# sangaprabhav/HypTokenizer

Hardware: AMD Instinct MI355X
Metric: merge_steps_per_sec (higher is better)
Workload: dtype bf16 prefilter + f32 canonical

## Files before the change

### hyptokenizer_amd/csrc/hm_engine.hip

```cpp
#include "hm_common.h"

static thread_local std::string g_last_error;

int hm_fail(hm_engine* e, int code, const std::string& msg)
{
    g_last_error = msg;
    if (e) e->err = msg;
    return code;
}

#define HM_WIDTH(v) v,
static const int kSupportedNG[] = {HM_SCAN_NG_LIST(HM_WIDTH, HM_SCAN_WIDTHS_ALL)};
static const int kSupportedKC[] = {HM_SCAN_KC_LIST(HM_WIDTH, HM_SCAN_WIDTHS_ALL)};
#undef HM_WIDTH

static int hm_pick_kc(int d)
{
    const int need = (d + 4 + 7) / 8;
    for (int v : kSupportedKC)
        if (v >= need) return v;
    return -1;
}

static int hm_pick_ng(int d)
{
    const int need = (d + 3) / 4;
    for (int v : kSupportedNG)
        if (v >= need) return v;
    return -1;
}

extern "C" int hm_abi_version(void) { return HM_ABI_VERSION; }

#if defined(HM_TUNING)
static const char* const kKnobNames[] = {"chunk", "tail", "tail_div", "big_rows", "shape", "incr_topk", "kc_even", "phases", "ph_share0", "ph_share1", "ph_share2", "ph_share3", "ph_share4",
                                        "ph_div1", "ph_div2", "ph_div3", "ph_div4", "ph_div5", "pipeline", "pipe_fault_at", "pipeline_pairs", "dyn", "dyn_slots", "head", "head_force", "head_ring", "head_span", "argmin_col_begin"};
#endif
static std::map<std::string, double> g_default_knobs;

static int hm_apply_knob(hm_engine* e, const char* name, double v)
{
    const std::string k = name ? name : "";
    if (k == "chunk") { if (!(v >= 4 && v <= 4096)) return HM_E_ARG; e->plan.chunk_f32 = e->plan.chunk_bf16 = (int)v; }
    else if (k == "tail") { if (!(v >= 0.0 && v <= 0.9)) return HM_E_ARG; e->plan.tail_fraction = v; }
    else if (k == "tail_div") { if (!(v >= 1 && v <= 16)) return HM_E_ARG; e->plan.tail_div = (int)v; }
    else if (k == "big_rows") { if (!(v >= 0)) return HM_E_ARG; e->plan.big_min_rows = (int64_t)v; }
    else if (k == "shape") { if (!(v >= -1 && v <= 4)) return HM_E_ARG; e->plan.force_shape = (int)v; }
    else if (k == "incr_topk") e->incremental_topk = v != 0.0;
    else if (k == "phases") { if (!(v >= 1 && v <= HM_SCAN_PHASES)) return HM_E_ARG; e->plan.phases = (int)v; }
    else if (k.size() == 9 && k.compare(0, 8, "ph_share") == 0 && k[8] >= '0' && k[8] < '0' + HM_SCAN_PHASES - 1) { if (!(v >= 0.0 && v <= 1.0)) return HM_E_ARG; e->plan.ph_share[k[8] - '0'] = v; }
    else if (k.size() == 7 && k.compare(0, 6, "ph_div") == 0 && k[6] >= '1' && k[6] < '0' + HM_SCAN_PHASES) { if (!(v >= 1 && v <= 64)) return HM_E_ARG; e->plan.ph_div[k[6] - '0'] = (int)v; }
    else if (k == "dyn_slots") { if (!(v >= 0 && v <= 65536)) return HM_E_ARG; e->dyn_slots = (int)v; }
    else if (k == "head") { if (!(v == 0.0 || v == (double)HM_SCAN_HEAD)) return HM_E_ARG; e->head = (int)v; }
    else if (k == "head_force") e->head_force = v != 0.0;
    else if (k == "head_ring") { if (!(v >= 0 && v < HM_SCAN_RINGS && v == (double)(int)v)) return HM_E_ARG; e->head_ring = (int)v; }
    else if (k == "head_span") { if (!(v == 1.0 || v == 2.0)) return HM_E_ARG; e->head_span = (int)v; }
    else if (k == "argmin_col_begin") { if (!(v >= 0)) return HM_E_ARG; e->argmin_col_begin = (int64_t)v; }
    else if (k == "expect_head_bad") { if (e->h == nullptr || (e->h->head_bad != 0u) != (v != 0.0)) return HM_E_STATE; return HM_OK; }
    else if (k == "dyn") e->dyn_queue = v != 0.0;
    else if (k == "pipeline") e->pipeline = v != 0.0;
    else if (k == "pipe_fault_at") e->pipe_fault_at = (int)v;
    else if (k == "exact_search") e->force_exact = v != 0.0;
    else if (k == "pipeline_pairs") { if (!(v >= 0)) return HM_E_ARG; e->pipeline_min_pairs = (int64_t)v; }
    else if (k == "kc_even") {
        if (e->img16 != nullptr) return HM_E_STATE;
        if (v != 0.0 && (e->KC & 1)) { e->KC += 1; e->RB16 = 16 * hm_row16_chunks(e->KC); }
    }
    else return HM_E_ARG;
    e->st.disarm();
    return HM_OK;
}

extern "C" int hm_debug_set_knob(hm_engine* e, const char* name, double value)
{
    if (!e) return hm_fail(nullptr, HM_E_ARG, "hm_debug_set_knob: engine is NULL");
    const int rc = hm_apply_knob(e, name, value);
    return rc ? hm_fail(e, rc, "hm_debug_set_knob: unknown knob or value out of range") : HM_OK;
}

extern "C" int hm_debug_set_default_knob(const char* name, double value, int clear)
{
    const std::string k = name ? name : "";
    if (clear) {
        if (k.empty()) { g_default_knobs.clear(); return hm_graph_default_knob(nullptr, 0.0, 1); }
        if (hm_graph_owns_knob(name)) return hm_graph_default_knob(name, 0.0, 1);
        g_default_knobs.erase(k);
        return HM_OK;
    }
    if (const int gk = hm_graph_default_knob(name, value, 0); gk <= 0)
        return gk ? hm_fail(nullptr, gk, "hm_debug_set_default_knob: unknown knob or value out of range") : HM_OK;
    hm_engine probe;
    const int rc = hm_apply_knob(&probe, name, value);
    if (rc) return hm_fail(nullptr, rc, "hm_debug_set_default_knob: unknown knob or value out of range");
    g_default_knobs[k] = value;
    return HM_OK;
}

extern "C" const char* hm_last_error(const hm_engine* e)
{
    if (e && !e->err.empty()) return e->err.c_str();
    return g_last_error.c_str();
}

static int hm_engine_alloc(hm_engine* e)
{
    const int device = e->device;
    HM_HIP(hipSetDevice(device));
    {
        int cus = 0;
        if (hipDeviceGetAttribute(&cus, hipDeviceAttributeMultiprocessorCount, device) == hipSuccess && cus > 0) e->n_cu = cus;
    }
    HM_HIP(hipMalloc(&e->img, sizeof(float) * (size_t)e->rows_alloc * e->RS));
    HM_HIP(hipMemset(e->img, 0, sizeof(float) * (size_t)e->rows_alloc * e->RS));
    HM_HIP(hipMalloc(&e->img16, (size_t)e->rows_alloc * e->RB16));
    HM_HIP(hipMemset(e->img16, 0, (size_t)e->rows_alloc * e->RB16));
    HM_HIP(hipMalloc(&e->ent, sizeof(uint4) * (size_t)e->ent_cap));
    HM_HIP(hipMalloc(&e->ent2, sizeof(uint4) * (size_t)e->ent_cap));
    HM_HIP(hipMalloc(&e->sorted, sizeof(uint4) * (size_t)e->sorted_cap));
    HM_HIP(hipMalloc(&e->d_prev, sizeof(uint4) * (size_t)e->sorted_cap));
    HM_HIP(hipMalloc(&e->d_batch, sizeof(int32_t) * 3 * HM_BATCH_MAX));
    HM_HIP(hipHostMalloc(&e->h_batch, sizeof(int32_t) * 3 * HM_BATCH_MAX, hipHostMallocDefault));
    HM_HIP(hipEventCreateWithFlags(&e->ev_batch, hipEventDisableTiming));
    HM_HIP(hipMalloc(&e->d_ctr, sizeof(uint32_t) * 8));
    HM_HIP(hipMemset(e->d_ctr, 0, sizeof(uint32_t) * 8));
    HM_HIP(hipMalloc(&e->d_rmax2_mem, sizeof(uint32_t) * 4));
    HM_HIP(hipMemset(e->d_rmax2_mem, 0, sizeof(uint32_t) * 4));
    e->d_rmax2 = e->d_rmax2_mem;
    HM_HIP(hipMalloc(&e->d_ctr64, sizeof(unsigned long long) * 8));
    HM_HIP(hipMemset(e->d_ctr64, 0, sizeof(unsigned long long) * 8));
    HM_HIP(hipMalloc(&e->d_queue, 256));
    HM_HIP(hipMemset(e->d_queue, 0, 256));
    HM_HIP(hipMalloc(&e->d_rowkey, sizeof(unsigned long long) * 3));
    HM_HIP(hipMemset(e->d_rowkey, 0xff, sizeof(unsigned long long) * 3));
    HM_HIP(hipMalloc(&e->d_seed, sizeof(ArgminSeed)));
    HM_HIP(hipMemset(e->d_seed, 0, sizeof(ArgminSeed)));
    HM_HIP(hipMalloc(&e->d_rec, 2 * sizeof(ArgminRec)));
    HM_HIP(hipMalloc(&e->d_loop_recs, HM_LOOP_MAX_STEPS * sizeof(ArgminRec)));
    HM_HIP(hipMalloc(&e->d_loop, sizeof(LoopState)));
// ... 222 lines not shown
```

### hyptokenizer_amd/csrc/hm_scan.hip

```cpp
#include <type_traits>

#include "hm_common.h"

#pragma clang fp contract(off)


template <int CNT>
__device__ __forceinline__ void hm_dma_group(const char* src, uint32_t dst)
{
    uint32_t keep;
    if constexpr (CNT == 4)
        asm volatile("s_mov_b32 %0, m0\n\ts_mov_b32 m0, %2\n\ts_nop 0\n\tglobal_load_lds_dwordx4 %1, off\n\t"
                     "global_load_lds_dwordx4 %1, off offset:1024\n\tglobal_load_lds_dwordx4 %1, off offset:2048\n\t"
                     "global_load_lds_dwordx4 %1, off offset:3072\n\ts_mov_b32 m0, %0"
                     : "=&s"(keep) : "v"(src), "s"(dst) : "memory");
    else if constexpr (CNT == 3)
        asm volatile("s_mov_b32 %0, m0\n\ts_mov_b32 m0, %2\n\ts_nop 0\n\tglobal_load_lds_dwordx4 %1, off\n\t"
                     "global_load_lds_dwordx4 %1, off offset:1024\n\tglobal_load_lds_dwordx4 %1, off offset:2048\n\t"
                     "s_mov_b32 m0, %0"
                     : "=&s"(keep) : "v"(src), "s"(dst) : "memory");
    else if constexpr (CNT == 2)
        asm volatile("s_mov_b32 %0, m0\n\ts_mov_b32 m0, %2\n\ts_nop 0\n\tglobal_load_lds_dwordx4 %1, off\n\t"
                     "global_load_lds_dwordx4 %1, off offset:1024\n\ts_mov_b32 m0, %0"
                     : "=&s"(keep) : "v"(src), "s"(dst) : "memory");
    else
        asm volatile("s_mov_b32 %0, m0\n\ts_mov_b32 m0, %2\n\ts_nop 0\n\tglobal_load_lds_dwordx4 %1, off\n\ts_mov_b32 m0, %0"
                     : "=&s"(keep) : "v"(src), "s"(dst) : "memory");
}

template <int PIECES, int FIRST = 0>
__device__ __forceinline__ void hm_dma_run(const char* src, uint32_t dst)
{
    if constexpr (FIRST < PIECES) {
        hm_dma_group<(PIECES - FIRST < 4 ? PIECES - FIRST : 4)>(src + FIRST * 1024, dst + FIRST * 1024u);
        hm_dma_run<PIECES, FIRST + 4>(src, dst);
    }
}

#ifndef HM_SCAN_PIPE_MAX_TM
#define HM_SCAN_PIPE_MAX_TM 2
#endif
#ifndef HM_SCAN_DEEP_PREFETCH
#define HM_SCAN_DEEP_PREFETCH 1
#endif
template <int NG, int SIGN, int MODE, int BF, int TM, int WPB, int SUB, bool WK = false, int HEAD = 0, int RING = 0, int SPAN = 1>
__global__ __launch_bounds__(64 * WPB, 2) void hm_scan_kernel(const ScanArgs p)
{
    static_assert(SUB % 2 == 0, "the two accumulator sets alternate between column groups: an even number per tile");
    static_assert(RING == 0 || HEAD > 0, "rings other than 0 belong to the head kernels");
    constexpr bool PIPE = (TM <= HM_SCAN_PIPE_MAX_TM);
    using G = ScanGeom<NG, BF, TM, WPB, SUB, RING, SPAN>;
    static_assert(G::SPAN == SPAN, "a span the ring has no slots for is the dispatch's to replace (hm_launch_scan_ng)");
    constexpr int COLS = G::COLS, RS = G::RS, RB16 = G::RB16, TILE_BYTES = G::TILE_BYTES, NP = G::NP;
    constexpr int PPW = G::PPW, TILE_LDS = G::TILE_LDS, DIST = G::DIST, NBUF = G::NBUF;
    constexpr int RSUB = G::RSUB;
    static_assert(RSUB % 2 == 0, "the head walk takes the groups of a slot in pairs");
    constexpr int WAVE_ROWS = G::WAVE_ROWS, BLOCK_ROWS = G::BLOCK_ROWS, NTHREADS = G::NTHREADS;
    constexpr bool HALF_LAST = (BF != 0) && (NG & 1);
    constexpr int TCH = RS / 4 - 1;
    static_assert(HEAD == 0 || (BF != 0 && SIGN != 0 && MODE == HM_MODE_ARGMIN && PIPE && HEAD == hm_head_steps(NG)),
                  "the head test: bf16 form, lorentz sign, argmin, two accumulator sets, the head set the image's r^ was built for");
    extern __shared__ __attribute__((aligned(16))) char smem[];

    if (p.stop != nullptr && *p.stop != 0u) return;
    if (p.order_seen != nullptr && __hip_atomic_load(p.order_seen, __ATOMIC_RELAXED, __HIP_MEMORY_SCOPE_AGENT) < p.order_need) {
        if (threadIdx.x == 0) __hip_atomic_store(p.order_fault, 5u, __ATOMIC_RELAXED, __HIP_MEMORY_SCOPE_AGENT);
        return;
    }

    const int lane = threadIdx.x & 63;
    const int wave = __builtin_amdgcn_readfirstlane(threadIdx.x >> 6);
    const int r = lane & 31, h = lane >> 5;

    uint32_t sure_total = 0;
    unsigned long long gk = ~0ull;
    unsigned long long gk_raw = ~0ull;
    bool gk_pending = false;
    const uint32_t lds_base = (uint32_t)(size_t)((__attribute__((address_space(3))) char*)smem);

    uint32_t* lhist = nullptr;
    if (MODE == HM_MODE_HIST) {
        lhist = reinterpret_cast<uint32_t*>(smem + G::HIST_OFF);
        for (int t = threadIdx.x; t < HM_HIST_BINS; t += NTHREADS) lhist[t] = 0;
    }

    int rb = 0, ct0 = 0, ct1 = 0, rb_cur = -1;
    int i0w = 0;
    bool wave_active = false, rows_full = false;

    const float delta = hm_scan_delta(BF != 0, BF ? 8 * NG : RS, p.rmax2_bits);
    const float pre_f = p.u_hi + delta;
    const float lo_f = p.u_lo - delta;
    const float zmax_f = 1.0f - delta;
    const bool cut_all = (p.cut_bits == 0xffffffffu);
    const float cut_f = cut_all ? p.u_hi : hm::bitsf(p.cut_bits) + delta;
    static_assert(!WK || MODE == HM_MODE_ARGMIN, "only the argmin search keeps a running key");
    const int key_si = WK ? p.key_si : 32 - HM_KEY_IB_NARROW, key_sj = WK ? p.key_sj : 2 * HM_KEY_IB_NARROW - 32;

    if (MODE == HM_MODE_ARGMIN) {
        const unsigned long long g0 = __hip_atomic_load(&p.ctr64[1], __ATOMIC_RELAXED, __HIP_MEMORY_SCOPE_AGENT);
        if (g0 < gk) gk = g0;
    }

    int hg_tot = 0, hc_tot = 0;

    float2 a[BF ? 1 : TM][BF ? 1 : NP];
    uint4 a16[BF ? TM : 1][BF ? NP : 1];
    uint4 a16t[HEAD ? TM : 1];
    auto frag_at = [&](const auto* base, int g) __attribute__((always_inline)) -> uint4 {
        const char* q = reinterpret_cast<const char*>(base);
        if (HALF_LAST && g == NP - 1) {
            const uint2 v = *reinterpret_cast<const uint2*>(q + 32 * g - 8 * h);
            return make_uint4(v.x, v.y, 0u, 0u);
        }
        return *reinterpret_cast<const uint4*>(q + 32 * g);
    };
    auto mfma16 = [&](const uint4& av, const uint4& bv, const f32x16& cv, int g) __attribute__((always_inline)) -> f32x16 {
        if (HALF_LAST && g == NP - 1) {
            typedef short s16x4 __attribute__((ext_vector_type(4)));
            const uint2 a2 = make_uint2(av.x, av.y), b2 = make_uint2(bv.x, bv.y);
            return __builtin_amdgcn_mfma_f32_32x32x8bf16_1k(__builtin_bit_cast(s16x4, a2), __builtin_bit_cast(s16x4, b2), cv, 0, 0, 0);
        }
        return __builtin_amdgcn_mfma_f32_32x32x16_bf16(__builtin_bit_cast(bf16x8, av), __builtin_bit_cast(bf16x8, bv), cv, 0, 0, 0);
    };
    auto load_a = [&]() __attribute__((always_inline)) {
    if constexpr (BF) {
#pragma unroll
        for (int tm = 0; tm < TM; ++tm) {
            const unsigned char* src = p.img16 + (int64_t)(i0w + 32 * tm + r) * RB16 + 16 * h;
#pragma unroll
            for (int g = 0; g < NP; ++g) a16[tm][g] = frag_at(src, g);
            if (h == 1) {
                const uint32_t z = HALF_LAST ? a16[tm][NP - 1].x : a16[tm][NP - 1].z;
                const uint32_t hi16 = z & 0xffffu, lo16 = z >> 16;
                const uint32_t t0 = (hi16 | (hi16 << 16)) ^ 0x80008000u, t1 = lo16 ^ 0x8000u;
// ... 306 lines not shown
                        ext = __builtin_fmaxf(ext, acc[set ^ 1][q / 16][q % 16]);
                }
            };
            kstep(std::integral_constant<int, 0>{});
            __builtin_amdgcn_sched_barrier(0);
            if constexpr (NEXT) {
#pragma unroll
                for (int k = 0; k < HEAD; ++k) bfr[set ^ 1][k] = frag_at(btn, hm_head_kstep(k, NP));
            }
            __builtin_amdgcn_sched_barrier(0);
            static_assert(HEAD <= 4, "the head k-steps are written out");
            if constexpr (HEAD > 1) kstep(std::integral_constant<int, 1>{});
            if constexpr (HEAD > 2) kstep(std::integral_constant<int, 2>{});
            if constexpr (HEAD > 3) kstep(std::integral_constant<int, 3>{});
            if constexpr (RED) ext = -ext;
        }
    };
    auto head_finish = [&](auto set_c, float ext_u, int buf, int sub, int j0s) __attribute__((always_inline)) -> bool {
        constexpr int set = decltype(set_c)::value;
        if constexpr (HEAD > 0) {
            float bound_f = pre_f;
            const uint32_t best_bits = (uint32_t)(gk >> 32);
            if (best_bits != 0xffffffffu) {
                const float bb = hm::bitsf(best_bits + hm_tie_slack(best_bits)) + 2.0f * delta;
                if (bb < bound_f) bound_f = bb;
            }
            if (__ballot(ext_u < bound_f) == 0ull) return false;
            const char* bt = smem + buf * TILE_LDS + (sub * 32 + r) * RB16 + 16 * h;
            const unsigned char* as = p.img16 + (int64_t)(i0w + r) * RB16 + 16 * h;
#pragma unroll
            for (int tm = 0; tm < TM; ++tm)
#pragma unroll
                for (int e = 0; e < 16; ++e) acc[set][tm][e] = 0.0f;
#pragma unroll 1
            for (int g = 0; g < NP - 1; ++g) {
                const uint4 bv = *reinterpret_cast<const uint4*>(bt + 32 * g);
#pragma unroll
                for (int tm = 0; tm < TM; ++tm) {
                    const uint4 av = *reinterpret_cast<const uint4*>(as + (int64_t)(32 * tm) * RB16 + 32 * g);
                    acc[set][tm] = __builtin_amdgcn_mfma_f32_32x32x16_bf16(__builtin_bit_cast(bf16x8, av), __builtin_bit_cast(bf16x8, bv), acc[set][tm], 0, 0, 0);
                }
            }
            {
                const uint4 bv = frag_at(bt, NP - 1);
#pragma unroll
                for (int tm = 0; tm < TM; ++tm) {
                    uint4 av = frag_at(as + (int64_t)(32 * tm) * RB16, NP - 1);
                    if (h == 1) {
                        const uint32_t z = HALF_LAST ? av.x : av.z;
                        const uint32_t hi16 = z & 0xffffu, lo16 = z >> 16;
                        const uint32_t t0 = (hi16 | (hi16 << 16)) ^ 0x80008000u, t1 = lo16 ^ 0x8000u;
                        if (HALF_LAST) { av.x = t0; av.y = t1; }
                        else { av.z = t0; av.w = t1; }
                    }
                    acc[set][tm] = mfma16(av, bv, acc[set][tm], NP - 1);
                }
            }
            finish_group(set_c, reduce_group(set_c), j0s);
            return true;
        }
        return false;
    };

    constexpr int WMAX = ScanRun::outstanding_max(NBUF, SPAN);
    auto ring_wait = [&](int tiles) __attribute__((always_inline)) {
        auto wait_p = [&](auto p_c) __attribute__((always_inline)) {
            constexpr int P = decltype(p_c)::value;
            static_assert(WMAX * P <= 60, "the counted wait must fit vmcnt");
            if (tiles >= 3 && WMAX >= 3) asm volatile("s_waitcnt vmcnt(%0)" : : "n"(3 * P) : "memory");
            else if (tiles >= 2 && WMAX >= 2) asm volatile("s_waitcnt vmcnt(%0)" : : "n"(2 * P) : "memory");
            else if (tiles >= 1 && WMAX >= 1) asm volatile("s_waitcnt vmcnt(%0)" : : "n"(P) : "memory");
            else asm volatile("s_waitcnt vmcnt(0)" : : : "memory");
        };
        static_assert(RING == 0 || WMAX <= 3, "ring_wait writes out the depths");
        if constexpr (PREM != 0) {
            if (wave < PREM) wait_p(std::integral_constant<int, PQ + 1>{});
            else wait_p(std::integral_constant<int, PQ>{});
        } else {
            wait_p(std::integral_constant<int, G::EXACT ? PQ : PPW>{});
        }
    };

    auto head_walk = [&](int buf, int j0) __attribute__((always_inline)) {
        if constexpr (HEAD > 0) {
            bool hp = false;
            int hg = 0, hc = 0;
#pragma unroll 1
            for (int sp = 0; sp < RSUB / 2; ++sp) {
                {
                    const int sub = 2 * sp;
                    const int j0s = j0 + sub * 32;
                    const bool do_c = wave_active && (j0s + 31 > i0w);
                    const char* bt = head_at(buf, sub);
                    float ext_u = 0.0f;
                    if (do_c && hp) {
                        head_group(std::integral_constant<int, 0>{}, std::true_type{}, std::true_type{}, bt, bt + 32 * RB16, false, ext_u);
                    } else {
                        if (do_c) head_group(std::integral_constant<int, 0>{}, std::false_type{}, std::true_type{}, bt, bt + 32 * RB16, true, ext_u);
                        if (hp) ext_u = reduce_group(std::integral_constant<int, 1>{});
                    }
                    if (hp) { ++hg; hc += head_finish(std::integral_constant<int, 1>{}, ext_u, buf, sub - 1, j0s - 32) ? 1 : 0; }
                    hp = do_c;
                }
                {
                    const int sub = 2 * sp + 1;
                    const int j0s = j0 + sub * 32;
                    const bool do_c = wave_active && (j0s + 31 > i0w);
                    const char* bt = head_at(buf, sub);
                    float ext_u = 0.0f;
                    if (do_c && hp) {
                        head_group(std::integral_constant<int, 1>{}, std::true_type{}, std::true_type{}, bt, bt + 32 * RB16, false, ext_u);
                    } else {
                        if (do_c) head_group(std::integral_constant<int, 1>{}, std::false_type{}, std::true_type{}, bt, bt + 32 * RB16, true, ext_u);
                        if (hp) ext_u = reduce_group(std::integral_constant<int, 0>{});
                    }
                    if (hp) { ++hg; hc += head_finish(std::integral_constant<int, 0>{}, ext_u, buf, sub - 1, j0s - 32) ? 1 : 0; }
                    hp = do_c;
                }
            }
            if (hp) { ++hg; hc += head_finish(std::integral_constant<int, 1>{}, reduce_group(std::integral_constant<int, 1>{}), buf, RSUB - 1, j0 + (RSUB - 1) * 32) ? 1 : 0; }
            hg_tot += hg; hc_tot += hc;
        }
    };

    auto head_tile_lean = [&](int buf0, int buf1, int j0) __attribute__((always_inline)) {
        if constexpr (HEAD > 0 && SPAN == 2) {
            static_assert(RSUB == 2, "two slots of two groups");
            float bound_f = pre_f;
            const uint32_t best_bits = (uint32_t)(gk >> 32);
            if (best_bits != 0xffffffffu) {
                const float bb = hm::bitsf(best_bits + hm_tie_slack(best_bits)) + 2.0f * delta;
                if (bb < bound_f) bound_f = bb;
            }
            const char* b0 = head_at(buf0, 0);
            const char* b1 = head_at(buf1, 0);
            float e0 = 0.0f, e1 = 0.0f, e2 = 0.0f;
            head_group(std::integral_constant<int, 0>{}, std::false_type{}, std::true_type{}, b0, b0 + 32 * RB16, true, e0);
            head_group(std::integral_constant<int, 1>{}, std::true_type{}, std::true_type{}, b0 + 32 * RB16, b1, false, e0);
            head_group(std::integral_constant<int, 0>{}, std::true_type{}, std::true_type{}, b1, b1 + 32 * RB16, false, e1);
            head_group(std::integral_constant<int, 1>{}, std::true_type{}, std::false_type{}, b1 + 32 * RB16, b1, false, e2);
            const float e3 = reduce_group(std::integral_constant<int, 1>{});
            hg_tot += 2 * RSUB;
            if (__ballot(__builtin_fminf(__builtin_fminf(e0, e1), __builtin_fminf(e2, e3)) < bound_f) != 0ull) {
#pragma unroll 1
                for (int g = 0; g < 2 * RSUB; ++g) {
                    const float eg = g == 0 ? e0 : (g == 1 ? e1 : (g == 2 ? e2 : e3));
                    hc_tot += head_finish(std::integral_constant<int, 0>{}, eg, g < RSUB ? buf0 : buf1, g % RSUB, j0 + 32 * g) ? 1 : 0;
                }
            }
        }
    };

    volatile uint32_t* const qslot = reinterpret_cast<volatile uint32_t*>(smem + G::queue_off(MODE));
    const bool dyn = (MODE != HM_MODE_HIST) && (p.dyn != 0);
    unsigned long long q_raw = 0ull;
    if (dyn && threadIdx.x == 0) (void)__hip_atomic_fetch_max(p.q_ctr, p.q_tag, __ATOMIC_RELAXED, __HIP_MEMORY_SCOPE_AGENT);
    int item = (int)blockIdx.x;
#pragma unroll 1
    for (;;) {
    bool have = true;
    HM_SCAN_ITEM_DECODE(p.items, item, BLOCK_ROWS, G::PLAN_COLS, p.nct, p.col_begin, rb, ct0, ct1)
    if constexpr (COLS != G::PLAN_COLS) {
        ct0 *= G::PLAN_COLS / COLS;
        ct1 *= G::PLAN_COLS / COLS;
        if (ct0 < p.col_begin / COLS) ct0 = p.col_begin / COLS;
        if (ct1 > (p.n + COLS - 1) / COLS) ct1 = (p.n + COLS - 1) / COLS;
    }
    if (ct0 >= ct1) have = false;

    int ct_step = 1;
    if (MODE == HM_MODE_HIST && have) {
        ct_step = p.sample_stride;
        ct0 += (ct_step - (ct0 + rb * 7) % ct_step) % ct_step;
        if (ct0 >= ct1) have = false;
    }
    if (have) {
    if (rb != rb_cur) {
        rb_cur = rb;
        i0w = rb * BLOCK_ROWS + wave * WAVE_ROWS;
        wave_active = (i0w < p.row_end) && (i0w + WAVE_ROWS - 1 >= p.row_begin) && (i0w < p.n);
        rows_full = (i0w >= p.row_begin) && (i0w + WAVE_ROWS - 1 < p.row_end);
        load_a();
    }
    const int ntile = (ct1 - ct0 + ct_step - 1) / ct_step;
    auto tile_at = [&](int t) { return ct0 + t * ct_step; };

    if constexpr (RING > 0) {
#pragma unroll
        for (int q = 0; q < NBUF - SPAN; ++q)
            if (q < ntile) dma_tile(tile_at(q), q);
        __builtin_amdgcn_s_waitcnt(0x0F70);
    } else {
#pragma unroll
    for (int q = 0; q < DIST; ++q) dma_tile(tile_at(q < ntile ? q : ntile - 1), q);
    if (DIST - 1 <= 0) asm volatile("s_waitcnt vmcnt(0)" ::: "memory");
    else asm volatile("s_waitcnt vmcnt(%0)" ::"n"((DIST - 1) * PPW) : "memory");
    if (DIST == 1) __builtin_amdgcn_s_waitcnt(0x0F70);
    }
    __syncthreads();

    bool pend = false;
    bool deep_valid = false;
    int pend_j0s = 0;
    int buf = 0;
    int gk_due = 0;

    if constexpr (SPAN == 2) {
        static_assert(HEAD > 0 && RING > 0 && MODE == HM_MODE_ARGMIN, "the span-2 walk is the head kernels'");
        const ScanRun run{ntile, NBUF, SPAN};
        const int ntk = run.tiles();
        const int j_right = rb * BLOCK_ROWS + BLOCK_ROWS;
        auto ring_add = [&](int b, int q) { b += q; return b >= NBUF ? b - NBUF : b; };
#pragma unroll 1
        for (int k = 0; k < ntk; ++k) {
            const int nslot = run.count(k);
            const int j0 = (ct0 + 2 * k) * COLS;
            const int buf1 = ring_add(buf, 1);
            const bool last = (k == ntk - 1);
            const bool poll = (k & 7) == 0;
            if (poll) asm volatile("global_load_dwordx2 v[252:253], %0, off sc1" : : "v"(&p.ctr64[1]) : "memory", "v252", "v253");
            if (dyn && last && threadIdx.x == 0)
                asm volatile("global_atomic_add_x2 v[254:255], %0, %1, off sc0" : : "v"(p.q_ctr), "v"(1ull) : "memory", "v254", "v255");
            {
                const int rq = run.req_first(k), nrq = run.req_count(k);
                const int bq = ring_add(buf, NBUF - SPAN);
                if (nrq > 0) dma_tile(ct0 + rq, bq);
                if (nrq > 1) dma_tile(ct0 + rq + 1, ring_add(bq, 1));
            }
            if (nslot == 2 && wave_active && j0 >= j_right) {
                head_tile_lean(buf, buf1, j0);
            } else {
#pragma unroll 1
                for (int sl = 0; sl < nslot; ++sl) head_walk(sl ? buf1 : buf, j0 + sl * COLS);
            }
            ring_wait(run.outstanding(k));
            if (poll) {
                uint32_t klo, khi;
                asm volatile("v_mov_b32 %0, v252\n\tv_mov_b32 %1, v253" : "=v"(klo), "=v"(khi) : : "memory", "v252", "v253");
                gk_raw = ((unsigned long long)khi << 32) | klo;
                if (gk_raw < gk) gk = gk_raw;
            }
            if (dyn && last && threadIdx.x == 0) {
                uint32_t qlo, qhi;
                asm volatile("v_mov_b32 %0, v254\n\tv_mov_b32 %1, v255" : "=v"(qlo), "=v"(qhi) : : "memory", "v254", "v255");
                qslot[0] = qlo; qslot[1] = qhi;
            }
            __syncthreads();
            buf = ring_add(buf, SPAN);
        }
    } else
    for (int t = 0; t < ntile; ++t) {
        const int ct = tile_at(t);
        const int ct_next = (t + DIST < ntile) ? tile_at(t + DIST) : ct;
        int buf_next = buf + DIST;
        if (buf_next >= NBUF) buf_next -= NBUF;
        const int j0 = ct * COLS;

        if (MODE == HM_MODE_ARGMIN && (t & (8 * (G::PLAN_COLS / COLS) - 1)) == 0) {
            if constexpr (RING > 0) {
                asm volatile("global_load_dwordx2 v[252:253], %0, off sc1" : : "v"(&p.ctr64[1]) : "memory", "v252", "v253");
                gk_due = t + DIST - 1;
            } else {
            asm volatile("global_load_dwordx2 %0, %1, off sc1" : "=v"(gk_raw) : "v"(&p.ctr64[1]) : "memory");
            }
            gk_pending = true;
        }
        if (dyn && t == ntile - 1 && threadIdx.x == 0) {
            if constexpr (RING > 0)
                asm volatile("global_atomic_add_x2 v[254:255], %0, %1, off sc0" : : "v"(p.q_ctr), "v"(1ull) : "memory", "v254", "v255");
            else
            asm volatile("global_atomic_add_x2 %0, %1, %2, off sc0" : "=v"(q_raw) : "v"(p.q_ctr), "v"(1ull) : "memory");
        }
        if constexpr (RING > 0) {
            if (t + DIST < ntile) dma_tile(ct_next, buf_next);
        } else {
        dma_tile(ct_next, buf_next);
        }

        if constexpr (HEAD > 0) {
            head_walk(buf, j0);
        } else if constexpr (!PIPE) {
            bool prev = false;
#pragma unroll 1
            for (int sub = 0; sub < SUB; ++sub) {
                const int j0s = j0 + sub * 32;
                const bool do_c = wave_active && (j0s + 31 > i0w);
                if (do_c) {
                    float ext_u = 0.0f;
                    mma_group(std::integral_constant<int, 0>{}, std::false_type{}, buf, sub, !prev, ext_u);
                    ext_u = reduce_group(std::integral_constant<int, 0>{});
                    finish_group(std::integral_constant<int, 0>{}, ext_u, j0s);
                }
                prev = do_c;
            }
        } else {
#pragma unroll 1
            for (int sp = 0; sp < SUB / 2; ++sp) {
                if constexpr (DEEP) {
                    const int ja = j0 + 2 * sp * 32, jb = ja + 32;
                    if (wave_active && (ja + 31 > i0w) && pend) {
                        float ea = 0.0f, eb = 0.0f;
                        mma_group_deep(std::integral_constant<int, 0>{}, buf, 2 * sp, !deep_valid, ea);
                        finish_group(std::integral_constant<int, 1>{}, ea, pend_j0s);
                        const bool more = 2 * sp + 2 < SUB;
                        mma_group_deep(std::integral_constant<int, 1>{}, buf, 2 * sp + 1, false, eb);
                        finish_group(std::integral_constant<int, 0>{}, eb, ja);
                        pend_j0s = jb;
                        deep_valid = more;
                        continue;
                    }
                    deep_valid = false;
                }
                {
                    const int sub = 2 * sp;
                    const int j0s = j0 + sub * 32;
                    const bool do_c = wave_active && (j0s + 31 > i0w);
                    float ext_u = 0.0f;
                    if (do_c && pend) {
                        mma_group(std::integral_constant<int, 0>{}, std::true_type{}, buf, sub, sp == 0, ext_u);
                    } else {
                        if (do_c) mma_group(std::integral_constant<int, 0>{}, std::false_type{}, buf, sub, true, ext_u);
                        if (pend) ext_u = reduce_group(std::integral_constant<int, 1>{});
                    }
                    if (pend) finish_group(std::integral_constant<int, 1>{}, ext_u, pend_j0s);
                    pend = do_c;
                    pend_j0s = j0s;
                }
                {
// ... 10 lines not shown
                    if (pend) finish_group(std::integral_constant<int, 0>{}, ext_u, pend_j0s);
                    pend = do_c;
                    pend_j0s = j0s;
                }
            }
        }

        if constexpr (RING > 0) {
            ring_wait(ntile - 2 - t);
            if (gk_pending && (t >= gk_due || t == ntile - 1)) {
                uint32_t klo, khi;
                asm volatile("v_mov_b32 %0, v252\n\tv_mov_b32 %1, v253" : "=v"(klo), "=v"(khi) : : "memory", "v252", "v253");
                gk_raw = ((unsigned long long)khi << 32) | klo;
                if (gk_raw < gk) gk = gk_raw;
                gk_pending = false;
            }
            if (dyn && t == ntile - 1 && threadIdx.x == 0) {
                uint32_t qlo, qhi;
                asm volatile("v_mov_b32 %0, v254\n\tv_mov_b32 %1, v255" : "=v"(qlo), "=v"(qhi) : : "memory", "v254", "v255");
                q_raw = ((unsigned long long)qhi << 32) | qlo;
            }
        } else {
        if (DIST - 1 <= 0) asm volatile("s_waitcnt vmcnt(0)" : "+v"(gk_raw), "+v"(q_raw) : : "memory");
        else asm volatile("s_waitcnt vmcnt(%2)" : "+v"(gk_raw), "+v"(q_raw) : "n"((DIST - 1) * PPW) : "memory");
        if (MODE == HM_MODE_ARGMIN && gk_pending) {
            if (gk_raw < gk) gk = gk_raw;
            gk_pending = false;
        }
        }
        if (dyn && t == ntile - 1 && threadIdx.x == 0) { qslot[0] = (uint32_t)q_raw; qslot[1] = (uint32_t)(q_raw >> 32); }
        __syncthreads();
        if (++buf == NBUF) buf = 0;
    }
    if constexpr (PIPE) {
        if (pend) {
            const float ext_u = reduce_group(std::integral_constant<int, 1>{});
            finish_group(std::integral_constant<int, 1>{}, ext_u, pend_j0s);
        }
    }

    if (DIST > 1 && RING == 0) { asm volatile("s_waitcnt vmcnt(0)" ::: "memory"); __syncthreads(); }
    }

    if (!dyn) break;
    if (!have) {
        __syncthreads();
        if (threadIdx.x == 0) {
            const unsigned long long v = __hip_atomic_fetch_add(p.q_ctr, 1ull, __ATOMIC_RELAXED, __HIP_MEMORY_SCOPE_AGENT);
            qslot[0] = (uint32_t)v; qslot[1] = (uint32_t)(v >> 32);
        }
        __syncthreads();
    }
    {
        const uint32_t qlo = __builtin_amdgcn_readfirstlane(qslot[0]), qhi = __builtin_amdgcn_readfirstlane(qslot[1]);
        const unsigned long long q = ((unsigned long long)qhi << 32) | qlo;
        if ((q >> 24) != (p.q_tag >> 24)) break;
        item = (int)gridDim.x + (int)(q & 0xffffffull);
        if (item >= p.n_items) break;
    }
    }

    if constexpr (HEAD > 0) {
        if (lane == 0 && hg_tot >= 16 && 2 * hc_tot > hg_tot) __hip_atomic_store(p.head_bad, 1u, __ATOMIC_RELAXED, __HIP_MEMORY_SCOPE_SYSTEM);
    }
    if (MODE == HM_MODE_TOPK) {
        unsigned long long s = sure_total;
#pragma unroll
        for (int off = 32; off > 0; off >>= 1) s += __shfl_xor(s, off, 64);
        if (lane == 0 && s != 0) atomicAdd(&p.ctr64[0], s);
    }
    if (MODE == HM_MODE_HIST) {
        __syncthreads();
        for (int t = threadIdx.x; t < HM_HIST_BINS; t += NTHREADS)
            if (lhist[t]) atomicAdd(&p.hist[t], lhist[t]);
    }
}

template <int NG, int SIGN, int MODE, int BF, int TM, int WPB, int SUB, bool WK = false, int HEAD = 0, int RING = 0, int SPAN = 1>
static hipError_t hm_launch_scan_t(hm_engine* e, const ScanArgs& a, dim3 grid, hipStream_t s, hipEvent_t ev0, hipEvent_t ev1)
{
    using G = ScanGeom<NG, BF, TM, WPB, SUB, RING, SPAN>;
    const size_t lds = G::lds_bytes(MODE);
    static_assert(RING == 0 || G::lds_bytes(MODE) <= HM_LDS_PER_BLOCK, "a deeper ring keeps two blocks per CU");
    const void* fn = reinterpret_cast<const void*>(&hm_scan_kernel<NG, SIGN, MODE, BF, TM, WPB, SUB, WK, HEAD, RING, SPAN>);
    if (lds > 48 * 1024 && e->attr_done.find(fn) == e->attr_done.end()) {
        hipError_t st = hipFuncSetAttribute(fn, hipFuncAttributeMaxDynamicSharedMemorySize, (int)lds);
        if (st != hipSuccess) return st;
        e->attr_done.insert(fn);
    }
    ScanArgs b = a;
    b.n_items = (int)grid.x;
    b.dyn = 0;
    if (e->dyn_queue && MODE != HM_MODE_HIST && grid.x < (1u << 24)) {
        auto it = e->scan_slots.find(fn);
        if (it == e->scan_slots.end()) {
            int per_cu = 0;
            hipError_t st = hipOccupancyMaxActiveBlocksPerMultiprocessor(&per_cu, fn, G::NTHREADS, lds);
            if (st != hipSuccess) return st;
            it = e->scan_slots.emplace(fn, std::max(1, per_cu) * e->n_cu).first;
        }
        const int slots = e->dyn_slots > 0 ? e->dyn_slots : it->second;
        if ((int)grid.x > slots) {
            grid.x = (unsigned)slots;
            b.dyn = 1;
            b.q_tag = (++e->scan_tag) << 24;
            b.q_ctr = e->d_queue + 16 * ((b.ctr64 == e->d_ctr64) ? 0 : 1);
        }
    }
    if (ev0 != nullptr || ev1 != nullptr) hipExtLaunchKernelGGL((hm_scan_kernel<NG, SIGN, MODE, BF, TM, WPB, SUB, WK, HEAD, RING, SPAN>), grid, dim3(G::NTHREADS), lds, s, ev0, ev1, 0, b);
    else hipLaunchKernelGGL((hm_scan_kernel<NG, SIGN, MODE, BF, TM, WPB, SUB, WK, HEAD, RING, SPAN>), grid, dim3(G::NTHREADS), lds, s, b);
    return hipGetLastError();
}

template <int NG, int BF, int TM, int WPB, int SUB>
static hipError_t hm_launch_scan_ng(hm_engine* e, int sign, int mode, const ScanArgs& a, dim3 grid, hipStream_t s, hipEvent_t ev0,
                                    hipEvent_t ev1)
{
    if (sign) {
        if (mode == HM_MODE_TOPK) return hm_launch_scan_t<NG, 1, HM_MODE_TOPK, BF, TM, WPB, SUB>(e, a, grid, s, ev0, ev1);
        if (mode == HM_MODE_ARGMIN) {
            constexpr int HD = (BF != 0 && TM <= HM_SCAN_PIPE_MAX_TM) ? hm_head_steps(NG) : 0;
            if constexpr (HD > 0) {
                if (hm_head_live(e)) {
#define HM_HEAD_RING_CASE(R, S)                                                                                            \
    case 4 * S + R: {                                                                                                      \
        constexpr int SP = ScanGeom<NG, BF, TM, WPB, SUB, R, S>::SPAN;                                                     \
        if (a.key_wide) return hm_launch_scan_t<NG, 1, HM_MODE_ARGMIN, BF, TM, WPB, SUB, true, HD, R, SP>(e, a, grid, s, ev0, ev1); \
        return hm_launch_scan_t<NG, 1, HM_MODE_ARGMIN, BF, TM, WPB, SUB, false, HD, R, SP>(e, a, grid, s, ev0, ev1);       \
    }
                    static_assert(HM_SCAN_RINGS == 3, "one case per ring and span");
                    switch (4 * (e->head_ring == 0 ? 1 : e->head_span) + e->head_ring) {
                        HM_HEAD_RING_CASE(0, 1) HM_HEAD_RING_CASE(1, 1) HM_HEAD_RING_CASE(2, 1) HM_HEAD_RING_CASE(1, 2) HM_HEAD_RING_CASE(2, 2)
                    }
#undef HM_HEAD_RING_CASE
                    return hipErrorInvalidValue;
                }
            }
            if (a.key_wide) return hm_launch_scan_t<NG, 1, HM_MODE_ARGMIN, BF, TM, WPB, SUB, true>(e, a, grid, s, ev0, ev1);
            return hm_launch_scan_t<NG, 1, HM_MODE_ARGMIN, BF, TM, WPB, SUB>(e, a, grid, s, ev0, ev1);
        }
        return hm_launch_scan_t<NG, 1, HM_MODE_HIST, BF, TM, WPB, SUB>(e, a, grid, s, ev0, ev1);
    }
    if (mode == HM_MODE_TOPK) return hm_launch_scan_t<NG, 0, HM_MODE_TOPK, BF, TM, WPB, SUB>(e, a, grid, s, ev0, ev1);
    if (mode == HM_MODE_ARGMIN) {
        if (a.key_wide) return hm_launch_scan_t<NG, 0, HM_MODE_ARGMIN, BF, TM, WPB, SUB, true>(e, a, grid, s, ev0, ev1);
        return hm_launch_scan_t<NG, 0, HM_MODE_ARGMIN, BF, TM, WPB, SUB>(e, a, grid, s, ev0, ev1);
    }
    return hm_launch_scan_t<NG, 0, HM_MODE_HIST, BF, TM, WPB, SUB>(e, a, grid, s, ev0, ev1);
}

bool hm_use_bf16(const hm_engine* e)
{
    if (!e->bf16_ok || e->force_f32) return false;
    if (e->precision == HM_PREFILTER_F32) return false;
    if (e->precision == HM_PREFILTER_BF16) return true;
    return e->d >= 24;
}

template <int S>
static hipError_t hm_launch_scan_bf16(hm_engine* e, int mode, const ScanArgs& a, dim3 grid, hipStream_t s, hipEvent_t ev0, hipEvent_t ev1)
{
    constexpr int TM = kScanShapes[S].tm, WPB = kScanShapes[S].wpb;
    static_assert(ScanGeom<13, 1, TM, WPB, HM_SUB_BF16>::BLOCK_ROWS == hm_shape_rows(S), "the item plan counts this shape's rows per block");
#define HM_KC_CASE(KCv)                                                                                                    \
    case KCv:                                                                                                              \
        if constexpr (S == 0 || KCv <= HM_SCAN_BIG_MAX_KC)                                                                 \
            return hm_launch_scan_ng<KCv, 1, TM, WPB, HM_SUB_BF16>(e, e->sign_mode, mode, a, grid, s, ev0, ev1);          \
        break;
    switch (e->KC) { HM_SCAN_KC_LIST(HM_KC_CASE, HM_SCAN_WIDTHS_BUILT) }
#undef HM_KC_CASE
    return hipErrorInvalidValue;
}

hipError_t hm_launch_scan(hm_engine* e, int mode, const ScanArgs& a, dim3 grid, hipStream_t s, hipEvent_t ev0, hipEvent_t ev1)
{
    if (a.bf16) {
        switch (a.shape) {
            case 0: return hm_launch_scan_bf16<0>(e, mode, a, grid, s, ev0, ev1);
            case 1: return hm_launch_scan_bf16<1>(e, mode, a, grid, s, ev0, ev1);
#if HM_SCAN_ALL_SHAPES
            case 2: return hm_launch_scan_bf16<2>(e, mode, a, grid, s, ev0, ev1);
            case 3: return hm_launch_scan_bf16<3>(e, mode, a, grid, s, ev0, ev1);
            case 4: return hm_launch_scan_bf16<4>(e, mode, a, grid, s, ev0, ev1);
#endif
        }
        return hipErrorInvalidValue;
    }
    constexpr int TM = kScanShapes[0].tm, WPB = kScanShapes[0].wpb;
#define HM_NG_CASE(NGv) case NGv: return hm_launch_scan_ng<NGv, 0, TM, WPB, HM_SUB_F32>(e, e->sign_mode, mode, a, grid, s, ev0, ev1);
    switch (e->NG) { HM_SCAN_NG_LIST(HM_NG_CASE, HM_SCAN_WIDTHS_BUILT) }
#undef HM_NG_CASE
    return hipErrorInvalidValue;
}

bool hm_prepare_scan(hm_engine* e, const Bounds& b, int64_t row_begin, int64_t row_end, ScanArgs& a, dim3& grid, int64_t n_limit,
                     int64_t col_begin, int mode)
{
    const int bf16 = hm_use_bf16(e) ? 1 : 0;
    const int head = (mode == HM_MODE_ARGMIN && bf16 && e->sign_mode && hm_head_steps(e->KC) > 0 && hm_head_live(e)) ? 1 : 0;
    const ScanPlan pl = hm_scan_plan(e->plan, ScanRequest{e->n, row_begin, row_end, n_limit, col_begin, bf16, e->KC, head});
    if (!pl.ok) return false;
    memset(&a, 0, sizeof(a));
    a.img = e->img;
    a.img16 = e->img16;
    a.bf16 = bf16;
    a.shape = pl.shape;
    a.n = pl.n;
    a.row_begin = pl.row_begin;
    a.row_end = pl.row_end;
    a.col_begin = pl.col_begin;
    a.rb_first = pl.rb_first;
    a.nct = pl.nct;
    a.items = pl.items;
    a.u_hi = b.u_hi;
    a.u_lo = b.u_lo;
// ... 19 lines not shown
```

### hyptokenizer_amd/csrc/hm_scan_geom.h

```cpp
#pragma once
#include "hm_tie_slack.h"

#define HM_MAX_BLOCK_ROWS 1024
#define HM_MODE_TOPK 0
#define HM_MODE_ARGMIN 1
#define HM_MODE_HIST 2
#define HM_HIST_BINS 256

#ifndef HM_SUB_BF16
#define HM_SUB_BF16 4
#endif
#ifndef HM_SUB_F32
#define HM_SUB_F32 2
#endif
#ifndef HM_DIST_BF16
#define HM_DIST_BF16 1
#endif
#ifndef HM_SCAN_INSTANTIATE_ALL
#define HM_SCAN_INSTANTIATE_ALL 1
#endif
#ifndef HM_SCAN_ALL_SHAPES
#define HM_SCAN_ALL_SHAPES 0
#endif

HM_HOST_DEVICE_INLINE constexpr int hm_row_floats(int NG) { return 4 * NG + 4 + (((NG + 1) % 2 == 0) ? 4 : 0); }
HM_HOST_DEVICE_INLINE constexpr int hm_row16_chunks(int KC) { return KC + ((KC & 1) ? 0 : 1); }

#define HM_SCAN_NG_LIST(X, REST) REST(X(1) X(2) X(3) X(4) X(6) X(8) X(10) X(13) X(16) X(20)) X(25) REST(X(28) X(32))
#define HM_SCAN_KC_LIST(X, REST) REST(X(2) X(4) X(8)) X(13) REST(X(14) X(16))
#define HM_SCAN_WIDTHS_ALL(...) __VA_ARGS__
#if HM_SCAN_INSTANTIATE_ALL
#define HM_SCAN_WIDTHS_BUILT(...) __VA_ARGS__
#else
#define HM_SCAN_WIDTHS_BUILT(...)
#endif

struct ScanShape { int tm, wpb; };
#define HM_SCAN_SHAPES 5
constexpr ScanShape kScanShapes[HM_SCAN_SHAPES] = {{2, 4}, {4, 4}, {2, 8}, {4, 8}, {3, 4}};
#define HM_SCAN_BIG_MAX_KC 14
HM_HOST_DEVICE_INLINE constexpr int hm_shape_rows(int shape) { return 32 * kScanShapes[shape].tm * kScanShapes[shape].wpb; }
HM_HOST_DEVICE_INLINE constexpr int hm_shape_rows_max(int shape = 0)
{
    return shape == HM_SCAN_SHAPES ? 0 : (hm_shape_rows(shape) > hm_shape_rows_max(shape + 1) ? hm_shape_rows(shape) : hm_shape_rows_max(shape + 1));
}
static_assert(hm_shape_rows_max() == HM_MAX_BLOCK_ROWS, "the images are allocated with one largest block of slack rows");

struct ScanRing { int sub, dist, exact; };
#define HM_SCAN_RINGS 3
constexpr ScanRing kScanRings[HM_SCAN_RINGS] = {{0, 0, 0}, {2, 3, 0}, {2, 4, 1}};
#define HM_SCAN_HEAD_RING_DEFAULT 1
#define HM_SCAN_HEAD_SPAN_DEFAULT 2
#define HM_LDS_PER_BLOCK (80 * 1024)

struct ScanRun {
    int ntile, nbuf, span;
    HM_HOST_DEVICE_INLINE constexpr int clamp(int s) const { return s < 0 ? 0 : (s > ntile ? ntile : s); }
    HM_HOST_DEVICE_INLINE constexpr int tiles() const { return (ntile + span - 1) / span; }
    HM_HOST_DEVICE_INLINE constexpr int prologue() const { return clamp(nbuf - span); }
    HM_HOST_DEVICE_INLINE constexpr int first(int k) const { return k * span; }
    HM_HOST_DEVICE_INLINE constexpr int count(int k) const { return clamp((k + 1) * span) - clamp(k * span); }
    HM_HOST_DEVICE_INLINE constexpr int req_first(int k) const { return clamp(nbuf + (k - 1) * span); }
    HM_HOST_DEVICE_INLINE constexpr int req_count(int k) const { return clamp(nbuf + k * span) - req_first(k); }
    HM_HOST_DEVICE_INLINE constexpr int outstanding(int k) const { return clamp(nbuf + k * span) - clamp((k + 2) * span); }
    HM_HOST_DEVICE_INLINE static constexpr int outstanding_max(int nbuf, int span) { return nbuf - 2 * span; }
};

template <int NG, int BF, int TM, int WPB, int SUB, int RING = 0, int SPAN_ASK = 1>
struct ScanGeom {
    static_assert(RING >= 0 && RING < HM_SCAN_RINGS && (RING == 0 || BF != 0), "rings other than 0: bf16 form");
    static constexpr int RSUB = kScanRings[RING].sub ? kScanRings[RING].sub : SUB;
    static constexpr bool EXACT = kScanRings[RING].exact != 0;
    static constexpr int PLAN_COLS = 32 * SUB;
    static constexpr int COLS = 32 * RSUB;
    static_assert(SUB % RSUB == 0, "an item's run of plan tiles is a whole number of ring tiles");
    static constexpr int RS = hm_row_floats(NG);
    static constexpr int RB16 = 16 * hm_row16_chunks(NG);
    static constexpr int ROW_BYTES = BF ? RB16 : RS * 4;
    static constexpr int TILE_BYTES = COLS * ROW_BYTES;
    static constexpr int NP = BF ? (NG + 1) / 2 : NG + 1;
    static constexpr int NPIECE = TILE_BYTES / 1024;
    static constexpr int PPW = (NPIECE + WPB - 1) / WPB;
    HM_HOST_DEVICE_INLINE static constexpr int wave_pieces(int w) { return EXACT ? NPIECE / WPB + (w < NPIECE % WPB ? 1 : 0) : PPW; }
    HM_HOST_DEVICE_INLINE static constexpr int wave_first(int w)
    {
        return EXACT ? w * (NPIECE / WPB) + (w < NPIECE % WPB ? w : NPIECE % WPB) : w * PPW;
    }
    static constexpr int TILE_LDS = EXACT ? TILE_BYTES : PPW * WPB * 1024;
    static constexpr int SLOTS_MAX = (HM_LDS_PER_BLOCK - 32 * ROW_BYTES - 16) / TILE_LDS;
    static constexpr int DIST = RING == 0 ? (BF ? HM_DIST_BF16 : 1)
                                          : (kScanRings[RING].dist + 1 <= SLOTS_MAX ? kScanRings[RING].dist : (SLOTS_MAX > 2 ? SLOTS_MAX - 1 : 1));
    static constexpr int NBUF = DIST + 1;
    static_assert(SPAN_ASK == 1 || SPAN_ASK == 2, "the walks that are written out");
    static constexpr int SPAN = (RING != 0 && NBUF >= 2 * SPAN_ASK) ? SPAN_ASK : 1;
    static_assert(SPAN == 1 || NBUF >= 2 * SPAN, "a compute tile's slots and the next one's are in the ring together");
    static constexpr int WAVE_ROWS = 32 * TM;
    static constexpr int BLOCK_ROWS = WPB * WAVE_ROWS;
    static constexpr int NTHREADS = 64 * WPB;
    static_assert(TILE_BYTES % 1024 == 0, "tiles are moved in 1 KiB pieces");
    static_assert(DIST * PPW <= 60, "the counted wait must fit vmcnt");
    static_assert(SPAN == 1 || ScanRun::outstanding_max(NBUF, SPAN) <= DIST - SPAN, "a span's waits leave less in flight than span 1's");

    static constexpr int RING_BYTES = NBUF * TILE_LDS;
    static constexpr int SLACK_BYTES = 32 * ROW_BYTES;
    static constexpr int HIST_OFF = RING_BYTES;
    static constexpr int QUEUE_BYTES = 16;
    HM_HOST_DEVICE_INLINE static constexpr int queue_off(int mode)
    {
        return RING_BYTES + SLACK_BYTES + (mode == HM_MODE_HIST ? 4 * HM_HIST_BINS : 0);
    }
    HM_HOST_DEVICE_INLINE static constexpr int lds_bytes(int mode) { return queue_off(mode) + QUEUE_BYTES; }
};
```

Before: 7039.

## Add a three-block-per-CU head ring and make it the default

Result: faster. 7287 (median of 6 runs) (+3.5%).

```diff
diff --git a/hyptokenizer_amd/csrc/hm_engine.hip b/hyptokenizer_amd/csrc/hm_engine.hip
--- a/hyptokenizer_amd/csrc/hm_engine.hip
+++ b/hyptokenizer_amd/csrc/hm_engine.hip
@@ -34,7 +34,7 @@
 
 #if defined(HM_TUNING)
 static const char* const kKnobNames[] = {"chunk", "tail", "tail_div", "big_rows", "shape", "incr_topk", "kc_even", "phases", "ph_share0", "ph_share1", "ph_share2", "ph_share3", "ph_share4",
-                                        "ph_div1", "ph_div2", "ph_div3", "ph_div4", "ph_div5", "pipeline", "pipe_fault_at", "pipeline_pairs", "dyn", "dyn_slots", "head", "head_force", "head_ring", "head_span", "argmin_col_begin"};
+                                        "ph_div1", "ph_div2", "ph_div3", "ph_div4", "ph_div5", "pipeline", "pipe_fault_at", "pipeline_pairs", "dyn", "dyn_slots", "head", "head_force", "head_ring", "head_blocks", "head_span", "argmin_col_begin"};
 #endif
 static std::map<std::string, double> g_default_knobs;
 
@@ -53,7 +53,8 @@
     else if (k == "dyn_slots") { if (!(v >= 0 && v <= 65536)) return HM_E_ARG; e->dyn_slots = (int)v; }
     else if (k == "head") { if (!(v == 0.0 || v == (double)HM_SCAN_HEAD)) return HM_E_ARG; e->head = (int)v; }
     else if (k == "head_force") e->head_force = v != 0.0;
-    else if (k == "head_ring") { if (!(v >= 0 && v < HM_SCAN_RINGS && v == (double)(int)v)) return HM_E_ARG; e->head_ring = (int)v; }
+    else if (k == "head_ring") { if (!(v >= 0 && v < HM_SCAN_RINGS_TWO_BLOCK && v == (double)(int)v)) return HM_E_ARG; e->head_ring = (int)v; }
+    else if (k == "head_blocks") { if (!(v == 2.0 || v == 3.0)) return HM_E_ARG; e->head_ring = v == 3.0 ? 3 : 1; }
     else if (k == "head_span") { if (!(v == 1.0 || v == 2.0)) return HM_E_ARG; e->head_span = (int)v; }
     else if (k == "argmin_col_begin") { if (!(v >= 0)) return HM_E_ARG; e->argmin_col_begin = (int64_t)v; }
     else if (k == "expect_head_bad") { if (e->h == nullptr || (e->h->head_bad != 0u) != (v != 0.0)) return HM_E_STATE; return HM_OK; }
diff --git a/hyptokenizer_amd/csrc/hm_scan.hip b/hyptokenizer_amd/csrc/hm_scan.hip
--- a/hyptokenizer_amd/csrc/hm_scan.hip
+++ b/hyptokenizer_amd/csrc/hm_scan.hip
@@ -44,13 +44,16 @@
 #define HM_SCAN_DEEP_PREFETCH 1
 #endif
 template <int NG, int SIGN, int MODE, int BF, int TM, int WPB, int SUB, bool WK = false, int HEAD = 0, int RING = 0, int SPAN = 1>
-__global__ __launch_bounds__(64 * WPB, 2) void hm_scan_kernel(const ScanArgs p)
+__global__ __launch_bounds__(64 * WPB, (HEAD > 0 && kScanRings[RING].blocks == 3) ? 3 : 2) void hm_scan_kernel(const ScanArgs p)
 {
     static_assert(SUB % 2 == 0, "the two accumulator sets alternate between column groups: an even number per tile");
     static_assert(RING == 0 || HEAD > 0, "rings other than 0 belong to the head kernels");
     constexpr bool PIPE = (TM <= HM_SCAN_PIPE_MAX_TM);
     using G = ScanGeom<NG, BF, TM, WPB, SUB, RING, SPAN>;
     static_assert(G::SPAN == SPAN, "a span the ring has no slots for is the dispatch's to replace (hm_launch_scan_ng)");
+    static_assert(G::RING == RING, "a ring the width or the span has no room for is the dispatch's to replace (hm_launch_scan_ng)");
+    constexpr bool TRI = (G::BLOCKS == 3);
+    static_assert(!TRI || (HEAD > 0 && SPAN == 2), "the three-block ring is the span-2 head kernels'");
     constexpr int COLS = G::COLS, RS = G::RS, RB16 = G::RB16, TILE_BYTES = G::TILE_BYTES, NP = G::NP;
     constexpr int PPW = G::PPW, TILE_LDS = G::TILE_LDS, DIST = G::DIST, NBUF = G::NBUF;
     constexpr int RSUB = G::RSUB;
@@ -523,7 +526,19 @@
     };
 
     auto head_walk = [&](int buf, int j0) __attribute__((always_inline)) {
-        if constexpr (HEAD > 0) {
+        if constexpr (TRI) {
+#pragma unroll 1
+            for (int sub = 0; sub < RSUB; ++sub) {
+                const int j0s = j0 + sub * 32;
+                if (!(wave_active && (j0s + 31 > i0w))) continue;
+                const char* bt = head_at(buf, sub);
+                float ext_u = 0.0f;
+                head_group(std::integral_constant<int, 0>{}, std::false_type{}, std::false_type{}, bt, bt, true, ext_u);
+                ext_u = reduce_group(std::integral_constant<int, 0>{});
+                ++hg_tot;
+                hc_tot += head_finish(std::integral_constant<int, 0>{}, ext_u, buf, sub, j0s) ? 1 : 0;
+            }
+        } else if constexpr (HEAD > 0) {
             bool hp = false;
             int hg = 0, hc = 0;
 #pragma unroll 1
@@ -659,9 +674,20 @@
             const int buf1 = ring_add(buf, 1);
             const bool last = (k == ntk - 1);
             const bool poll = (k & 7) == 0;
+            unsigned long long k_raw = ~0ull, d_raw = 0ull;
+            if constexpr (TRI) {
+                if (poll) k_raw = __hip_atomic_load(&p.ctr64[1], __ATOMIC_RELAXED, __HIP_MEMORY_SCOPE_AGENT);
+                if (dyn && last && threadIdx.x == 0) {
+                    uint64_t qa = reinterpret_cast<uint64_t>(p.q_ctr);
+                    asm volatile("" : "+v"(qa));
+                    d_raw = __hip_atomic_fetch_add(reinterpret_cast<__attribute__((address_space(1))) unsigned long long*>(qa), 1ull, __ATOMIC_RELAXED,
+                                                   __HIP_MEMORY_SCOPE_AGENT);
+                }
+            } else {
             if (poll) asm volatile("global_load_dwordx2 v[252:253], %0, off sc1" : : "v"(&p.ctr64[1]) : "memory", "v252", "v253");
             if (dyn && last && threadIdx.x == 0)
                 asm volatile("global_atomic_add_x2 v[254:255], %0, %1, off sc0" : : "v"(p.q_ctr), "v"(1ull) : "memory", "v254", "v255");
+            }
             {
                 const int rq = run.req_first(k), nrq = run.req_count(k);
                 const int bq = ring_add(buf, NBUF - SPAN);
@@ -674,6 +700,11 @@
 #pragma unroll 1
                 for (int sl = 0; sl < nslot; ++sl) head_walk(sl ? buf1 : buf, j0 + sl * COLS);
             }
+            if constexpr (TRI) {
+                asm volatile("s_waitcnt vmcnt(0)" : "+v"(k_raw), "+v"(d_raw) : : "memory");
+                if (k_raw < gk) gk = k_raw;
+                if (dyn && last && threadIdx.x == 0) { qslot[0] = (uint32_t)d_raw; qslot[1] = (uint32_t)(d_raw >> 32); }
+            } else {
             ring_wait(run.outstanding(k));
             if (poll) {
                 uint32_t klo, khi;
@@ -685,6 +716,7 @@
                 uint32_t qlo, qhi;
                 asm volatile("v_mov_b32 %0, v254\n\tv_mov_b32 %1, v255" : "=v"(qlo), "=v"(qhi) : : "memory", "v254", "v255");
                 qslot[0] = qlo; qslot[1] = qhi;
+            }
             }
             __syncthreads();
             buf = ring_add(buf, SPAN);
@@ -861,6 +893,7 @@
     using G = ScanGeom<NG, BF, TM, WPB, SUB, RING, SPAN>;
     const size_t lds = G::lds_bytes(MODE);
     static_assert(RING == 0 || G::lds_bytes(MODE) <= HM_LDS_PER_BLOCK, "a deeper ring keeps two blocks per CU");
+    static_assert(G::BLOCKS != 3 || 3 * hm_lds_alloc(G::lds_bytes(MODE)) <= HM_LDS_PER_CU, "a three-block ring keeps three");
     const void* fn = reinterpret_cast<const void*>(&hm_scan_kernel<NG, SIGN, MODE, BF, TM, WPB, SUB, WK, HEAD, RING, SPAN>);
     if (lds > 48 * 1024 && e->attr_done.find(fn) == e->attr_done.end()) {
         hipError_t st = hipFuncSetAttribute(fn, hipFuncAttributeMaxDynamicSharedMemorySize, (int)lds);
@@ -903,13 +936,14 @@
                 if (hm_head_live(e)) {
 #define HM_HEAD_RING_CASE(R, S)                                                                                            \
     case 4 * S + R: {                                                                                                      \
-        constexpr int SP = ScanGeom<NG, BF, TM, WPB, SUB, R, S>::SPAN;                                                     \
-        if (a.key_wide) return hm_launch_scan_t<NG, 1, HM_MODE_ARGMIN, BF, TM, WPB, SUB, true, HD, R, SP>(e, a, grid, s, ev0, ev1); \
-        return hm_launch_scan_t<NG, 1, HM_MODE_ARGMIN, BF, TM, WPB, SUB, false, HD, R, SP>(e, a, grid, s, ev0, ev1);       \
-    }
-                    static_assert(HM_SCAN_RINGS == 3, "one case per ring and span");
+        constexpr int RG = ScanGeom<NG, BF, TM, WPB, SUB, R, S>::RING, SP = ScanGeom<NG, BF, TM, WPB, SUB, R, S>::SPAN; \
+        if (a.key_wide) return hm_launch_scan_t<NG, 1, HM_MODE_ARGMIN, BF, TM, WPB, SUB, true, HD, RG, SP>(e, a, grid, s, ev0, ev1); \
+        return hm_launch_scan_t<NG, 1, HM_MODE_ARGMIN, BF, TM, WPB, SUB, false, HD, RG, SP>(e, a, grid, s, ev0, ev1);      \
+    }
+                    static_assert(HM_SCAN_RINGS == 4, "one case per ring and span");
                     switch (4 * (e->head_ring == 0 ? 1 : e->head_span) + e->head_ring) {
-                        HM_HEAD_RING_CASE(0, 1) HM_HEAD_RING_CASE(1, 1) HM_HEAD_RING_CASE(2, 1) HM_HEAD_RING_CASE(1, 2) HM_HEAD_RING_CASE(2, 2)
+                        HM_HEAD_RING_CASE(0, 1) HM_HEAD_RING_CASE(1, 1) HM_HEAD_RING_CASE(2, 1) HM_HEAD_RING_CASE(3, 1)
+                        HM_HEAD_RING_CASE(1, 2) HM_HEAD_RING_CASE(2, 2) HM_HEAD_RING_CASE(3, 2)
                     }
 #undef HM_HEAD_RING_CASE
                     return hipErrorInvalidValue;
diff --git a/hyptokenizer_amd/csrc/hm_scan_geom.h b/hyptokenizer_amd/csrc/hm_scan_geom.h
--- a/hyptokenizer_amd/csrc/hm_scan_geom.h
+++ b/hyptokenizer_amd/csrc/hm_scan_geom.h
@@ -46,10 +46,14 @@
 }
 static_assert(hm_shape_rows_max() == HM_MAX_BLOCK_ROWS, "the images are allocated with one largest block of slack rows");
 
-struct ScanRing { int sub, dist, exact; };
-#define HM_SCAN_RINGS 3
-constexpr ScanRing kScanRings[HM_SCAN_RINGS] = {{0, 0, 0}, {2, 3, 0}, {2, 4, 1}};
-#define HM_SCAN_HEAD_RING_DEFAULT 1
+struct ScanRing { int sub, dist, exact, blocks; };
+#define HM_SCAN_RINGS 4
+#define HM_SCAN_RINGS_TWO_BLOCK 3
+constexpr ScanRing kScanRings[HM_SCAN_RINGS] = {{0, 0, 0, 0}, {2, 3, 0, 0}, {2, 4, 1, 0}, {2, 3, 1, 3}};
+#define HM_LDS_PER_CU (160 * 1024)
+#define HM_LDS_GRANULE 1280
+HM_HOST_DEVICE_INLINE constexpr int hm_lds_alloc(int bytes) { return (bytes + HM_LDS_GRANULE - 1) / HM_LDS_GRANULE * HM_LDS_GRANULE; }
+#define HM_SCAN_HEAD_RING_DEFAULT 3
 #define HM_SCAN_HEAD_SPAN_DEFAULT 2
 #define HM_LDS_PER_BLOCK (80 * 1024)
 
@@ -66,17 +70,22 @@
     HM_HOST_DEVICE_INLINE static constexpr int outstanding_max(int nbuf, int span) { return nbuf - 2 * span; }
 };
 
-template <int NG, int BF, int TM, int WPB, int SUB, int RING = 0, int SPAN_ASK = 1>
+template <int NG, int BF, int TM, int WPB, int SUB, int RING_ASK = 0, int SPAN_ASK = 1>
 struct ScanGeom {
-    static_assert(RING >= 0 && RING < HM_SCAN_RINGS && (RING == 0 || BF != 0), "rings other than 0: bf16 form");
+    static_assert(RING_ASK >= 0 && RING_ASK < HM_SCAN_RINGS && (RING_ASK == 0 || BF != 0), "rings other than 0: bf16 form");
+    static constexpr int RS = hm_row_floats(NG);
+    static constexpr int RB16 = 16 * hm_row16_chunks(NG);
+    static constexpr int ROW_BYTES = BF ? RB16 : RS * 4;
+    static constexpr int QUEUE_BYTES = 16;
+    static constexpr int ASK_BLOCKS = kScanRings[RING_ASK].blocks;
+    static constexpr int ASK_LDS = (kScanRings[RING_ASK].dist + 1) * 32 * kScanRings[RING_ASK].sub * ROW_BYTES + QUEUE_BYTES;
+    static constexpr int RING = (ASK_BLOCKS == 3 && !(SPAN_ASK == 2 && 3 * hm_lds_alloc(ASK_LDS) <= HM_LDS_PER_CU)) ? 1 : RING_ASK;
+    static constexpr int BLOCKS = kScanRings[RING].blocks ? kScanRings[RING].blocks : 2;
     static constexpr int RSUB = kScanRings[RING].sub ? kScanRings[RING].sub : SUB;
     static constexpr bool EXACT = kScanRings[RING].exact != 0;
     static constexpr int PLAN_COLS = 32 * SUB;
     static constexpr int COLS = 32 * RSUB;
     static_assert(SUB % RSUB == 0, "an item's run of plan tiles is a whole number of ring tiles");
-    static constexpr int RS = hm_row_floats(NG);
-    static constexpr int RB16 = 16 * hm_row16_chunks(NG);
-    static constexpr int ROW_BYTES = BF ? RB16 : RS * 4;
     static constexpr int TILE_BYTES = COLS * ROW_BYTES;
     static constexpr int NP = BF ? (NG + 1) / 2 : NG + 1;
     static constexpr int NPIECE = TILE_BYTES / 1024;
@@ -89,7 +98,7 @@
     static constexpr int TILE_LDS = EXACT ? TILE_BYTES : PPW * WPB * 1024;
     static constexpr int SLOTS_MAX = (HM_LDS_PER_BLOCK - 32 * ROW_BYTES - 16) / TILE_LDS;
     static constexpr int DIST = RING == 0 ? (BF ? HM_DIST_BF16 : 1)
-                                          : (kScanRings[RING].dist + 1 <= SLOTS_MAX ? kScanRings[RING].dist : (SLOTS_MAX > 2 ? SLOTS_MAX - 1 : 1));
+                                          : (BLOCKS == 3 || kScanRings[RING].dist + 1 <= SLOTS_MAX ? kScanRings[RING].dist : (SLOTS_MAX > 2 ? SLOTS_MAX - 1 : 1));
     static constexpr int NBUF = DIST + 1;
     static_assert(SPAN_ASK == 1 || SPAN_ASK == 2, "the walks that are written out");
     static constexpr int SPAN = (RING != 0 && NBUF >= 2 * SPAN_ASK) ? SPAN_ASK : 1;
@@ -102,12 +111,14 @@
     static_assert(SPAN == 1 || ScanRun::outstanding_max(NBUF, SPAN) <= DIST - SPAN, "a span's waits leave less in flight than span 1's");
 
     static constexpr int RING_BYTES = NBUF * TILE_LDS;
-    static constexpr int SLACK_BYTES = 32 * ROW_BYTES;
+    static constexpr int SLACK_BYTES = BLOCKS == 3 ? 0 : 32 * ROW_BYTES;
     static constexpr int HIST_OFF = RING_BYTES;
-    static constexpr int QUEUE_BYTES = 16;
     HM_HOST_DEVICE_INLINE static constexpr int queue_off(int mode)
     {
         return RING_BYTES + SLACK_BYTES + (mode == HM_MODE_HIST ? 4 * HM_HIST_BINS : 0);
     }
     HM_HOST_DEVICE_INLINE static constexpr int lds_bytes(int mode) { return queue_off(mode) + QUEUE_BYTES; }
+    static_assert(BLOCKS != 3 || (EXACT && NBUF == 4 && SPAN == 2 && RING_BYTES + QUEUE_BYTES == 4 * TILE_BYTES + 16), "a three-block ring: four exact slots and the queue word");
+    static_assert(BLOCKS != 3 || 3 * hm_lds_alloc(RING_BYTES + QUEUE_BYTES) <= HM_LDS_PER_CU, "three blocks, each rounded up to the allocation granule, fit a CU's LDS");
+    static_assert(BLOCKS != 3 || ScanRun::outstanding_max(NBUF, SPAN) == 0, "a three-block ring: every tile wait is vmcnt(0)");
 };
```
